# ZikangYuan/sr_livo

Hardware: AMD Instinct MI355X
Metric: sweeps/s (full ESIKF solve of a 64k-pt Livox sweep vs 1M-pt voxel map) (higher is better)
Workload: dtype f64; 1 GPU; HEADLINE: stream of 4 distinct 65536-keypoint livox sweeps (own poses and priors), 978481-pt voxel map (1000000 target), max_num_residuals=2147483647, r=1, K=20; one full ESIKF solve per sweep, every sweep crosses PCIe once (uploaded on the copy stream during the solve before it: resident in HBM when its solve starts); sweeps drawn with seeds 20251309 + 100 j, keeping those that take sweep 0's 2 E; parallelism=single GPU

## Files before the change

### sr_livo_amd/csrc/srl_capi.cpp

```cpp
#include "../../include/srlivo_hip.h"
#include "../../include/srlivo_hip_debug.h"
#include "host/srl_la.h"
#include "srl_device.h"
#include "srl_hash.h"
#include "srl_heap.h"

#include <hip/hip_runtime.h>
#include <sched.h>

#include <algorithm>
#include <atomic>
#include <chrono>
#include <climits>
#include <cstdio>
#include <cstdlib>
#include <cstring>
#include <mutex>
#include <string>
#include <vector>

struct SrlMapState;
int srl_map_insert_device(struct srl_ctx *ctx, const double *world_xyz, int n, double voxel_size, int cap,
                          double min_distance_points, int min_num_points, int *num_added);

// ... 135 lines not shown
    ctx->counted = true;
    *out = ctx;
    return SRL_OK;
}

int srl_ctx_destroy(srl_ctx *ctx) {
    if (!ctx) return SRL_OK;
    hipSetDevice(ctx->device);
    if (ctx->counted && ctx->device < SRL_MAX_DEVICES) g_live_ctx[ctx->device].fetch_sub(1, std::memory_order_relaxed);
    if (ctx->armed.on) srl_ctx_disarm(ctx);
    if (ctx->stream) hipStreamSynchronize(ctx->stream);
    if (ctx->copy_stream) hipStreamSynchronize(ctx->copy_stream);
    if (ctx->color) srl_color_map_destroy(ctx);
    if (ctx->flow) srl_flow_destroy(ctx);
    if (ctx->prep) srl_image_prep_destroy(ctx);
    srl_consensus_release(ctx);
    if (ctx->pose_box_pinned) hipHostFree(ctx->pose_box_pinned);
    if (ctx->pose_box_dev) hipFree(ctx->pose_box_dev);
    if (ctx->d_pose_relay) hipFree(ctx->d_pose_relay);
    if (ctx->comm && srl_rccl()) srl_rccl()->CommDestroy(ctx->comm);
    if (ctx->parked_comm && srl_rccl()) srl_rccl()->CommDestroy(ctx->parked_comm);
    if (ctx->d_sub_kept) hipFree(ctx->d_sub_kept);
    if (ctx->d_sub_seen) hipFree(ctx->d_sub_seen);
    void *bufs[] = {ctx->d_corr_in, ctx->d_corr_rel, ctx->d_corr_imu, ctx->d_corr_raw, ctx->d_corr_seg, ctx->d_frame_raw, ctx->d_frame_world, ctx->d_table, ctx->d_slabs, ctx->cur.soa, ctx->d_rec, ctx->d_status, ctx->d_partials, ctx->d_binfo,
                    ctx->d_out, ctx->d_count, ctx->d_bound, ctx->d_granules, ctx->d_rec_granules, ctx->next.soa, ctx->next.stage, ctx->cur.stage, ctx->d_tap_ids, ctx->d_tap_ncand, ctx->d_tap_normal, ctx->d_tap_a2d,
                    ctx->d_tap_offset, ctx->d_gather, ctx->d_peer, ctx->d_mail};
    for (int r = 0; r < SRL_MAX_PEERS; r++) if (ctx->peer_mapped[r]) hipIpcCloseMemHandle(ctx->peer_mapped[r]);
    if (ctx->d_inbox) hipFree(ctx->d_inbox);
    for (void *b : bufs) if (b) hipFree(b);
    if (ctx->h_out) hipHostFree(ctx->h_out);
    if (ctx->h_count) hipHostFree(ctx->h_count);
    if (ctx->h_mail) hipHostFree(ctx->h_mail);
    if (ctx->h_arm_stamps) hipHostFree(ctx->h_arm_stamps);
    if (ctx->h_scratch) hipHostFree(ctx->h_scratch);
    if (ctx->h_frame_x) hipHostFree(ctx->h_frame_x);
    for (SrlEpochTable *t : {&ctx->sel_table, &ctx->ins_table}) { if (t->keyw) hipFree(t->keyw); if (t->minw) hipFree(t->minw); }
    if (ctx->d_frame_sync) hipFree(ctx->d_frame_sync);
    if (ctx->d_tr1_sched) hipFree(ctx->d_tr1_sched);
    if (ctx->h_insert_cnt) hipHostFree(ctx->h_insert_cnt);
    if (ctx->ev_insert) hipEventDestroy(ctx->ev_insert);
    if (ctx->ev_world) hipEventDestroy(ctx->ev_world);
    if (ctx->ev_frame_read) hipEventDestroy(ctx->ev_frame_read);
    if (ctx->h_chunks) { hipHostFree(ctx->h_chunks); for (int i = 0; i < srl_ctx::CHUNK_SLOTS; i++) if (ctx->chunk_ev[i]) hipEventDestroy(ctx->chunk_ev[i]); }
    for (auto &b : ctx->pool_free) hipFree(b.p);
    ctx->pool_free.clear();
    for (int i = 0; i < 4; i++) if (ctx->ev[i]) hipEventDestroy(ctx->ev[i]);
    for (SrlProfRing::Entry &e : ctx->prof.e) for (int k = 0; k < 2; k++) if (e.ev[k]) hipEventDestroy(e.ev[k]);
    for (int sl = 0; sl < 2; sl++) for (int k = 0; k < 2; k++) if (ctx->up_ev[sl][k]) hipEventDestroy(ctx->up_ev[sl][k]);
    if (ctx->upload_ev) hipEventDestroy(ctx->upload_ev);
    if (ctx->copy_stream) { hipStreamSynchronize(ctx->copy_stream); hipStreamDestroy(ctx->copy_stream); }
    if (ctx->prefix_stream) { hipStreamSynchronize(ctx->prefix_stream); hipStreamDestroy(ctx->prefix_stream); }
    if (ctx->stream) hipStreamDestroy(ctx->stream);
    delete ctx;
    return SRL_OK;
}

const char *srl_last_error(const srl_ctx *ctx) { return ctx ? ctx->err.c_str() : "null context"; }

int srl_map_upload(srl_ctx *ctx, const int16_t *keys_xyz, const int32_t *counts, const float *xyz, int V, int cap) {
    if (!ctx || V < 0 || (V > 0 && (!keys_xyz || !counts || !xyz))) return SRL_ERR_BAD_ARG;
    SRL_DISARM(ctx);
    if (cap != SRL_VOXEL_CAP) { ctx->err = "max_num_points_in_voxel must be 20"; return SRL_ERR_UNSUPPORTED; }
    HIPCHK(ctx, hipSetDevice(ctx->device));
    { const int rcs = srl_map_settle(ctx); if (rcs) return rcs; }
    ctx->bound_n = 0;
    const unsigned slab_cap = std::max<unsigned>(1024u, (unsigned)V + (unsigned)V / 2u + 4096u);
    if (slab_cap > SRL_MAX_SLABS) { ctx->err = "map too large: slab byte offsets are 32-bit (16.7 M voxels)"; return SRL_ERR_UNSUPPORTED; }
    const unsigned table_cap = next_pow2(std::max<unsigned>(2048u, SRL_TABLE_FACTOR * slab_cap));
    std::vector<SrlSlab> slabs((size_t)V);
    std::vector<SrlMapSlot> table((size_t)table_cap);
    for (auto &s : table) { s.key = SRL_EMPTY_KEY; s.slab = 0; s.count = 0; }
    long long npts = 0;
    const unsigned mask = table_cap - 1;
    for (int v = 0; v < V; v++) {
        SrlSlab &s = slabs[v];
        std::memset(&s, 0, sizeof s);
        const int c = counts[v];
        if (c < 0 || c > cap) { ctx->err = "voxel count out of range"; return SRL_ERR_BAD_ARG; }
        for (int i = 0; i < c; i++)
            for (int d = 0; d < 3; d++) s.xyz[i][d] = xyz[((size_t)v * cap + i) * 3 + d];
        s.count = (unsigned)c;
        s.key = srl_pack_key(keys_xyz[3 * v], keys_xyz[3 * v + 1], keys_xyz[3 * v + 2]);
        npts += c;
        unsigned h = srl_hash_key(s.key) & mask;
        while (table[h].key != SRL_EMPTY_KEY) {
            if (table[h].key == s.key) { ctx->err = "duplicate voxel key in upload"; return SRL_ERR_BAD_ARG; }
            h = (h + 1) & mask;
        }
        table[h].key = s.key;
        table[h].slab = (unsigned)v;
        table[h].count = (unsigned)c;
    }
    if (ctx->d_slabs) { HIPCHK(ctx, hipFree(ctx->d_slabs)); ctx->d_slabs = nullptr; }
    if (ctx->d_table) { HIPCHK(ctx, hipFree(ctx->d_table)); ctx->d_table = nullptr; }
    HIPCHK(ctx, hipMalloc((void **)&ctx->d_slabs, ((size_t)slab_cap + 1) * SRL_SLAB_BYTES));
    HIPCHK(ctx, hipMemsetD32Async((hipDeviceptr_t)(ctx->d_slabs + (size_t)slab_cap * SRL_SLAB_BYTES), 0x7f800000, SRL_SLAB_BYTES / 4, ctx->stream));
    HIPCHK(ctx, hipMalloc((void **)&ctx->d_table, (size_t)table_cap * sizeof(SrlMapSlot)));
    HIPCHK(ctx, hipMemsetAsync(ctx->d_slabs, 0, (size_t)slab_cap * SRL_SLAB_BYTES, ctx->stream));
    if (V > 0) HIPCHK(ctx, hipMemcpyAsync(ctx->d_slabs, slabs.data(), (size_t)V * SRL_SLAB_BYTES, hipMemcpyHostToDevice, ctx->stream));
    HIPCHK(ctx, hipMemcpyAsync(ctx->d_table, table.data(), (size_t)table_cap * sizeof(SrlMapSlot), hipMemcpyHostToDevice, ctx->stream));
    HIPCHK(ctx, hipStreamSynchronize(ctx->stream));
    ctx->slab_cap = slab_cap;
    ctx->table_cap = table_cap;
    ctx->num_voxels = V;
    ctx->num_points = npts;
    return SRL_OK;
}

int srl_map_size(srl_ctx *ctx, int64_t *num_points, int32_t *num_voxels) {
    if (!ctx) return SRL_ERR_BAD_ARG;
    { const int rcs = srl_map_settle(ctx); if (rcs) return rcs; }
    if (num_points) *num_points = ctx->num_points;
    if (num_voxels) *num_voxels = ctx->num_voxels;
    return SRL_OK;
}

int srl_map_download(srl_ctx *ctx, int16_t *keys_xyz, int32_t *counts, float *xyz, int max_voxels) {
    if (!ctx) return SRL_ERR_BAD_ARG;
    SRL_DISARM(ctx);
    if (!ctx->d_slabs) return SRL_ERR_NO_MAP;
    { const int rcs = srl_map_settle(ctx); if (rcs) return rcs; }
    const int V = ctx->num_voxels;
    if (max_voxels < V) return SRL_ERR_BAD_ARG;
    HIPCHK(ctx, hipSetDevice(ctx->device));
    std::vector<SrlSlab> slabs((size_t)V);
    if (V > 0) HIPCHK(ctx, hipMemcpyAsync(slabs.data(), ctx->d_slabs, (size_t)V * SRL_SLAB_BYTES, hipMemcpyDeviceToHost, ctx->stream));
    HIPCHK(ctx, hipStreamSynchronize(ctx->stream));
    for (int v = 0; v < V; v++) {
        short x, y, z;
        srl_unpack_key(slabs[v].key, &x, &y, &z);
        if (keys_xyz) { keys_xyz[3 * v] = x; keys_xyz[3 * v + 1] = y; keys_xyz[3 * v + 2] = z; }
        if (counts) counts[v] = (int32_t)slabs[v].count;
        if (xyz)
            for (int i = 0; i < SRL_CAP; i++)
                for (int d = 0; d < 3; d++)
                    xyz[((size_t)v * SRL_CAP + i) * 3 + d] = (i < (int)slabs[v].count) ? slabs[v].xyz[i][d] : 0.0f;
    }
    return SRL_OK;
}

int srl_map_insert(srl_ctx *ctx, const double *world_xyz, int n, double voxel_size, int cap,
                   double min_distance_points, int min_num_points, int *num_added) {
    if (!ctx || n < 0 || (n > 0 && !world_xyz)) return SRL_ERR_BAD_ARG;
    SRL_DISARM(ctx);
    if (cap != SRL_VOXEL_CAP) { ctx->err = "max_num_points_in_voxel must be 20"; return SRL_ERR_UNSUPPORTED; }
    return srl_map_insert_device(ctx, world_xyz, n, voxel_size, cap, min_distance_points, min_num_points, num_added);
}

int srl_map_insert_report(srl_ctx *ctx, const double *world_xyz, int n, double voxel_size, int cap, double min_distance_points, int min_num_points,
                          double ref_z, uint8_t *outcome, srl_cloud_point *cloud, int *num_cloud, int *num_added) {
    if (num_cloud) *num_cloud = 0;
    if (num_added) *num_added = 0;
    if (!ctx || n < 0 || (n > 0 && !world_xyz)) return SRL_ERR_BAD_ARG;
    SRL_DISARM(ctx);
    if (cap != SRL_VOXEL_CAP) { ctx->err = "max_num_points_in_voxel must be 20"; return SRL_ERR_UNSUPPORTED; }
    return srl_map_insert_report_device(ctx, world_xyz, n, voxel_size, cap, min_distance_points, min_num_points, ref_z, outcome, cloud, num_cloud, num_added);
}

namespace {
int upload_aos(srl_ctx *ctx, const char *src, size_t bytes, double *d_stage, hipStream_t st, bool last = true, int pinned = -1) {
    if (pinned < 0 ? srl_is_pinned(src) : pinned != 0) {
        HIPCHK(ctx, hipMemcpyAsync(d_stage, src, bytes, hipMemcpyHostToDevice, st));
        if (last) {
            if (!ctx->upload_ev) HIPCHK(ctx, hipEventCreateWithFlags(&ctx->upload_ev, hipEventDisableTiming));
            HIPCHK(ctx, hipEventRecord(ctx->upload_ev, st));
            ctx->upload_pending = true;
        }
        return SRL_OK;
    }
    int rc2 = upload_chunks_init(ctx);
    if (rc2) return rc2;
// ... 1547 lines not shown
```

### sr_livo_amd/csrc/srl_hash.h

```cpp
#pragma once
#include <stdint.h>
#ifdef __HIPCC__
#define SRL_HD __host__ __device__
#else
#define SRL_HD
#endif

SRL_HD inline unsigned long long srl_pack_key(short x, short y, short z) {
    return (unsigned long long)(unsigned short)x | ((unsigned long long)(unsigned short)y << 16) |
           ((unsigned long long)(unsigned short)z << 32);
}
SRL_HD inline void srl_unpack_key(unsigned long long k, short *x, short *y, short *z) {
    *x = (short)(unsigned short)(k & 0xFFFFu);
    *y = (short)(unsigned short)((k >> 16) & 0xFFFFu);
    *z = (short)(unsigned short)((k >> 32) & 0xFFFFu);
}
SRL_HD inline unsigned srl_hash_key(unsigned long long k) {
    const unsigned x = (unsigned)(k & 0xFFFFu), y = (unsigned)((k >> 16) & 0xFFFFu), z = (unsigned)((k >> 32) & 0xFFFFu);
#ifdef __HIP_DEVICE_COMPILE__
    unsigned h = __umul24(x, 0x9E3779u) ^ __umul24(y, 0x85EBCBu) ^ __umul24(z, 0xC2B2AFu);
#else
    unsigned h = (x * 0x9E3779u) ^ (y * 0x85EBCBu) ^ (z * 0xC2B2AFu);
#endif
    h ^= h >> 15;
    h *= 0x2C1B3C6Du;
    h ^= h >> 12;
    return h;
}
```

### sr_livo_amd/csrc/srl_kernels.hip

```cpp
#include "srl_device.h"
#include "srl_hash.h"
#include "srl_heap.h"

#include <math.h>
#include <type_traits>

namespace {

struct alignas(8) VoxEnt { unsigned slab; unsigned count; };
struct Surv { double d2; float x, y, z; unsigned id; };
static_assert(sizeof(Surv) == 24, "survivor record is 24 bytes");
static_assert(SRL_SURV_CAP * 24 + (SRL_MAXK + 1) * 8 <= SRL_WAVE_SCRATCH, "general-path scratch (survivors + sorted d2) must fit");
static_assert(64 * 8 + SRL_MAXK * 16 + SRL_MAXK * 4 <= SRL_WAVE_SCRATCH, "heap replay scratch must fit");

__device__ __forceinline__ int lane_id() {
    return __builtin_amdgcn_mbcnt_hi(~0u, __builtin_amdgcn_mbcnt_lo(~0u, 0));
}
__device__ __forceinline__ int lanes_below(unsigned long long m) {
    return __builtin_amdgcn_mbcnt_hi((unsigned)(m >> 32), __builtin_amdgcn_mbcnt_lo((unsigned)m, 0));
}

struct Cand { bool valid; double d2; float x, y, z; unsigned id; };

__device__ __forceinline__ Cand eval_cand(int e, int nv, const VoxEnt *vox, const unsigned char *slabs,
                                          double qx, double qy, double qz) {
    Cand c;
    c.valid = false;
    c.d2 = __builtin_huge_val();
    c.x = c.y = c.z = 0.0f;
    c.id = 0;
    const unsigned cv = (unsigned)e / SRL_CAP;
    const unsigned slot = (unsigned)e - cv * SRL_CAP;
    if ((int)cv < nv) {
        const VoxEnt ve = vox[cv];
        if (slot < ve.count) {
            const float *p = reinterpret_cast<const float *>(slabs + (size_t)ve.slab * SRL_SLAB_BYTES + slot * 12u);
            c.x = p[0]; c.y = p[1]; c.z = p[2];
            const double dx = (double)c.x - qx;
            const double dy = (double)c.y - qy;
            const double dz = (double)c.z - qz;
            c.d2 = (dx * dx + dy * dy) + dz * dz;
            c.valid = true;
            c.id = ve.slab * SRL_CAP + slot;
        }
    }
    return c;
}

template <int NB>
__device__ __forceinline__ int probe_voxels(double qx, double qy, double qz, double size_voxel, int thr_cap,
                                            const SrlMapSlot *table, unsigned mask, VoxEnt *vox, int lane, const float *qf_cull = nullptr,
                                            int *total_all = nullptr) {
    constexpr int SIDE = 2 * NB + 1;
    constexpr int NV = SIDE * SIDE * SIDE;
    asm volatile("" : "+v"(lane));
    const short kx = (short)(int)(qx / size_voxel);
    const short ky = (short)(int)(qy / size_voxel);
    const short kz = (short)(int)(qz / size_voxel);
    int nv = 0, tot = 0;
#pragma unroll
    for (int base = 0; base < NV; base += 64) {
        const int i = base + lane;
        bool found = false;
        unsigned slab = 0, cnt = 0;
        float bd2 = 0.0f;
        if (i < NV) {
            const int ix = i / (SIDE * SIDE);
            const int iy = (i / SIDE) % SIDE;
            const int iz = i % SIDE;
            const short vx = (short)(kx + (ix - NB));
            const short vy = (short)(ky + (iy - NB));
            const short vz = (short)(kz + (iz - NB));
            const unsigned long long key = srl_pack_key(vx, vy, vz);
            unsigned h = srl_hash_key(key) & mask;
            for (unsigned probe = 0; probe <= mask; ++probe) {
                const SrlMapSlot s = table[h];
                if (s.key == key) {
                    found = (int)s.count >= thr_cap && s.count > 0;
                    slab = s.slab;
                    cnt = s.count;
                    break;
                }
                if (s.key == SRL_EMPTY_KEY) break;
                h = (h + 1) & mask;
            }
            if (qf_cull) {
                const int vv[3] = {(int)vx, (int)vy, (int)vz};
                const float sz = (float)size_voxel;
#pragma unroll
                for (int ax = 0; ax < 3; ++ax) {
                    const int v = vv[ax];
                    const float lo = (float)(v > 0 ? v : v - 1) * sz, hi = (float)(v < 0 ? v : v + 1) * sz;
                    const float d = fmaxf(fmaxf(lo - qf_cull[ax], qf_cull[ax] - hi), 0.0f);
                    bd2 += d * d;
                }
            }
        }
        tot += found ? (int)cnt : 0;
        if (qf_cull) found = found && bd2 <= qf_cull[5];
        const unsigned long long m = __ballot(found);
        if (found) {
            VoxEnt ve; ve.slab = slab; ve.count = cnt;
            vox[nv + lanes_below(m)] = ve;
        }
        nv += __popcll(m);
    }
    if (total_all) {
        for (int d = 32; d >= 1; d >>= 1) tot += __shfl_xor(tot, d);
        *total_all = tot;
    }
    __builtin_amdgcn_wave_barrier();
    return nv;
}

enum { SEL_OVERFLOW = 0, SEL_DONE = 1, SEL_TIE = 2 };
#define SRL_NEAR_TIE 0x1.0000000000004p+0

template <class Sink>
__device__ __forceinline__ void select_topk_replay(double qx, double qy, double qz, int nv, const VoxEnt *vox,
                                                const unsigned char *slabs, int K, void *scratch, int lane, Sink &sink,
                                                int &total_out) {
    double *stage = reinterpret_cast<double *>(scratch);
    double *hd = stage + 64;
    int *he = reinterpret_cast<int *>(hd + SRL_MAXK);
    int *out = he + SRL_MAXK;
    const int rounds = (nv * SRL_CAP + 63) >> 6;
    int size = 0, total = 0;
    __builtin_amdgcn_wave_barrier();
    for (int j = 0; j < rounds; ++j) {
        const Cand c = eval_cand(lane + 64 * j, nv, vox, slabs, qx, qy, qz);
        stage[lane] = c.valid ? sqrt(c.d2) : -1.0;
        total += __popcll(__ballot(c.valid));
        __builtin_amdgcn_wave_barrier();
        if (lane == 0) {
            for (int i = 0; i < 64; ++i) {
                const double d = stage[i];
                if (d >= 0.0) size = srl_heap_offer(hd, he, size, K, d, 64 * j + i);
            }
        }
        __builtin_amdgcn_wave_barrier();
    }
    if (lane == 0) srl_heap_drain(hd, he, size, out);
    __builtin_amdgcn_wave_barrier();
    size = __shfl(size, 0);
    if (lane < size) {
        const Cand c = eval_cand(out[lane], nv, vox, slabs, qx, qy, qz);
        sink.put(lane, c.x, c.y, c.z, c.id);
    }
    total_out = total;
    __builtin_amdgcn_wave_barrier();
}

template <class Sink>
__device__ __forceinline__ void select_topk(double qx, double qy, double qz, int nv, const VoxEnt *vox,
                                            const unsigned char *slabs, int K, int select_mode, Surv *surv,
                                            int lane, Sink &sink, int &total_out, int &fallback_out) {
    const int rounds = (nv * SRL_CAP + 63) >> 6;
    const float kInfF = __builtin_huge_valf();
    asm volatile("" : "+v"(lane));
    if (select_mode == 5) {
        select_topk_replay(qx, qy, qz, nv, vox, slabs, K, surv, lane, sink, total_out);
        fallback_out = 1;
        return;
    }

    float lmin = kInfF;
    int total = 0;
// ... 44 lines not shown

    if (!use_fallback) {
        const int i = lane;
        const bool act = i < c_surv;
        Surv me;
        if (act) me = surv[i];
        else { me.d2 = __builtin_huge_val(); me.x = me.y = me.z = 0.0f; me.id = 0; }
        int rank = 0;
        for (int j = 0; j < c_surv; ++j) {
            const double dj = surv[j].d2;
            rank += ((dj < me.d2) || (dj == me.d2 && j < i)) ? 1 : 0;
        }
        if (act && rank <= K) sorted[rank] = me.d2;
        __builtin_amdgcn_wave_barrier();
        bool bad = false;
        if (act && rank < K && rank + 1 < c_surv) bad = !(sorted[rank + 1] > me.d2 * SRL_NEAR_TIE);
        tie = __ballot(bad) != 0ull;
        if (!tie && act && rank < K) sink.put(rank, me.x, me.y, me.z, me.id);
        fallback_out = 0;
    } else {
        double last_d2 = -1.0;
        int last_e = -1;
        const int next = total < K + 1 ? total : K + 1;
        for (int r = 0; r < next; ++r) {
            double bd2 = __builtin_huge_val();
            int be = 0x7fffffff;
            for (int j = 0; j < rounds; ++j) {
                const int e = lane + 64 * j;
                const Cand c = eval_cand(e, nv, vox, slabs, qx, qy, qz);
                const bool gt = c.valid && (c.d2 > last_d2 || (c.d2 == last_d2 && e > last_e));
                if (gt && (c.d2 < bd2 || (c.d2 == bd2 && e < be))) { bd2 = c.d2; be = e; }
            }
#pragma unroll
            for (int off = 32; off >= 1; off >>= 1) {
                const double od = __shfl_xor(bd2, off);
                const int oe = __shfl_xor(be, off);
                if (od < bd2 || (od == bd2 && oe < be)) { bd2 = od; be = oe; }
            }
            if (r > 0 && !(bd2 > last_d2 * SRL_NEAR_TIE)) { tie = true; break; }
            if (r < nsel && (be & 63) == lane) {
                const Cand c = eval_cand(be, nv, vox, slabs, qx, qy, qz);
                sink.put(r, c.x, c.y, c.z, c.id);
            }
            last_d2 = bd2;
            last_e = be;
        }
        fallback_out = 1;
    }
    __builtin_amdgcn_wave_barrier();
    if (tie) {
        select_topk_replay(qx, qy, qz, nv, vox, slabs, K, surv, lane, sink, total_out);
        fallback_out = 1;
    }
}

struct LaneRole {
    int pdx, pdy, pdz;
    int c0, slot;
};
__device__ __forceinline__ LaneRole lane_role(int lane) {
    LaneRole r;
    const int pl = lane & 31;
    const int ix = pl / 9, iy = (pl / 3) % 3, iz = pl % 3;
    r.pdx = ix - 1; r.pdy = iy - 1; r.pdz = iz - 1;
    r.c0 = lane / SRL_CAP;
    r.slot = lane - r.c0 * SRL_CAP;
    return r;
}

struct ProbeReq {
    unsigned long long key;
    unsigned h;
    SrlMapSlot s0, s1;
};
__device__ __forceinline__ ProbeReq probe_issue(const int *kv, int kl, const LaneRole &role, const SrlMapSlot *table,
                                                unsigned mask, int lane) {
    ProbeReq r;
    r.key = SRL_EMPTY_KEY; r.h = 0;
    r.s0.key = SRL_EMPTY_KEY; r.s0.slab = 0; r.s0.count = 0;
    r.s1 = r.s0;
    if ((lane & 31) < 27) {
        const int *k = kv + (kl + (lane >> 5)) * 4;
        r.key = srl_pack_key((short)(k[0] + role.pdx), (short)(k[1] + role.pdy), (short)(k[2] + role.pdz));
        r.h = srl_hash_key(r.key) & mask;
        r.s0 = table[r.h];
        r.s1 = table[(r.h + 1) & mask];
    }
    return r;
}
__device__ __forceinline__ int probe_finish(const ProbeReq &r, int thr_cap, const SrlMapSlot *table, unsigned mask,
                                            VoxEnt *vox, int lane, int *ncand_pair, bool cull = false, const float *qf_pair = nullptr,
                                            const int *kv_pair = nullptr, const LaneRole *role = nullptr, float size_voxel = 1.0f) {
    const bool prober = (lane & 31) < 27;
    const bool m0 = prober && r.s0.key == r.key;
    const bool m1 = prober && !m0 && r.s0.key != SRL_EMPTY_KEY && r.s1.key == r.key;
    bool found = m0 || m1;
    unsigned slab = m0 ? r.s0.slab : r.s1.slab, cnt = m0 ? r.s0.count : r.s1.count;
    const bool more = prober && !found && r.s0.key != SRL_EMPTY_KEY && r.s1.key != SRL_EMPTY_KEY;
    if (__ballot(more) != 0ull) {
        if (more) {
            unsigned h = (r.h + 2) & mask;
            for (unsigned probe = 2; probe <= mask; ++probe) {
                const SrlMapSlot sl = table[h];
                if (sl.key == r.key) { slab = sl.slab; cnt = sl.count; found = true; break; }
                if (sl.key == SRL_EMPTY_KEY) break;
                h = (h + 1) & mask;
            }
        }
    }
    found = found && (int)cnt >= thr_cap && cnt > 0;
    {
#if defined(__HIP_DEVICE_COMPILE__)
        int v = found ? (int)cnt : 0;
        v += __builtin_amdgcn_update_dpp(0, v, 0x111, 0xF, 0xF, false);
        v += __builtin_amdgcn_update_dpp(0, v, 0x112, 0xF, 0xF, false);
        v += __builtin_amdgcn_update_dpp(0, v, 0x114, 0xF, 0xF, false);
        v += __builtin_amdgcn_update_dpp(0, v, 0x118, 0xF, 0xF, false);
        v += __builtin_amdgcn_update_dpp(0, v, 0x142, 0xA, 0xF, false);
        if ((lane & 31) == 31) ncand_pair[lane >> 5] = v;
#endif
    }
    if (cull) {
        const int hh = lane >> 5;
        const float *qf = qf_pair + 8 * hh;
        const int *kv = kv_pair + 4 * hh;
        const float r2 = qf[5];
        float bd2 = 0.0f;
        const int pd[3] = {role->pdx, role->pdy, role->pdz};
#pragma unroll
        for (int ax = 0; ax < 3; ++ax) {
            const int v = kv[ax] + pd[ax];
            const float lo = (float)(v > 0 ? v : v - 1) * size_voxel, hi = (float)(v < 0 ? v : v + 1) * size_voxel;
            const float d = fmaxf(fmaxf(lo - qf[ax], qf[ax] - hi), 0.0f);
            bd2 += d * d;
        }
        found = found && bd2 <= r2;
    }
    const unsigned long long m = __ballot(found);
    const unsigned m_lo = (unsigned)m, m_hi = (unsigned)(m >> 32);
    const int nv_a = __popc(m_lo), nv_b = __popc(m_hi);
    if (prober) {
        const bool upper = lane >= 32;
        const unsigned f_lo = found ? m_lo : (~m_lo & 0x7FFFFFFu), f_hi = found ? m_hi : (~m_hi & 0x7FFFFFFu);
        const int below = upper ? (int)__builtin_amdgcn_mbcnt_hi(f_hi, 0u) : (int)__builtin_amdgcn_mbcnt_lo(f_lo, 0u);
        const int nv_own = upper ? nv_b : nv_a;
        VoxEnt ve; ve.slab = found ? slab : 0u; ve.count = found ? cnt : 0u;
        vox[(upper ? 32 : 0) + (found ? below : nv_own + below)] = ve;
    }
    __builtin_amdgcn_wave_barrier();
    return nv_a | (nv_b << 8);
}

struct LdsSink {
    float *col;
    int row;
    int plane;
    int *tap_ids;
    __device__ __forceinline__ void put(int rank, float x, float y, float z, unsigned id) {
        float *p = col + rank * row;
        p[0] = x;
        p[plane] = y;
        p[2 * plane] = z;
        if (tap_ids) tap_ids[rank] = (int)id;
    }
};

struct alignas(16) SurvRec { float x, y, z; int code; };
#define SRL_PAIR_MAX_ROUNDS 4

__device__ __forceinline__ float d2_f32(float px, float py, float pz, float qx, float qy, float qz) {
#pragma clang fp contract(fast)
    const float dx = px - qx, dy = py - qy, dz = pz - qz;
    return dx * dx + dy * dy + dz * dz;
}

template <class Sink>
__device__ __forceinline__ int finish_survivors(double qx, double qy, double qz, int c, const VoxEnt *vox, int K, void *scratch,
                                                int lane, Sink &sink, double *tau_out = nullptr) {
    SurvRec *recs = reinterpret_cast<SurvRec *>(__builtin_assume_aligned(scratch, 16));
    double *keys = reinterpret_cast<double *>(reinterpret_cast<unsigned char *>(scratch) + 1024);
    double *sorted = keys + 66;
    __builtin_amdgcn_wave_barrier();
    const bool act = lane < c;
    SurvRec me;
    me.x = me.y = me.z = 0.0f; me.code = 0;
    double my = __builtin_huge_val();
    if (act) {
        me = recs[lane];
        const double dx = (double)me.x - qx;
// ... 1990 lines not shown
```

### sr_livo_amd/csrc/srl_map_kernels.hip

```cpp
#include "srl_ctx.h"
#include "srl_frame_scratch.h"
#include "srl_hash.h"


#include <cstring>
#include <vector>

namespace {


template <bool XF>
__global__ void k_point_slots(const double *xyz, int n, double voxel_size, unsigned long long *keyw, unsigned mask, unsigned epoch16, unsigned *slot_out,
                              unsigned *idx, int *new_flag, const SrlFrameTransform T) {
    const int i = blockIdx.x * blockDim.x + threadIdx.x;
    if (i >= n) return;
    double wx, wy, wz;
    if (XF) {
        srl_transform_point(T.X, T.raw[(size_t)i * 3], T.raw[(size_t)i * 3 + 1], T.raw[(size_t)i * 3 + 2], wx, wy, wz);
        T.world[(size_t)i * 3] = wx; T.world[(size_t)i * 3 + 1] = wy; T.world[(size_t)i * 3 + 2] = wz;
    } else {
        wx = xyz[(size_t)i * 3]; wy = xyz[(size_t)i * 3 + 1]; wz = xyz[(size_t)i * 3 + 2];
    }
    const float fx = (float)wx, fy = (float)wy, fz = (float)wz;
    const short kx = (short)(int)((double)fx / voxel_size);
    const short ky = (short)(int)((double)fy / voxel_size);
    const short kz = (short)(int)((double)fz / voxel_size);
    const unsigned long long key = srl_pack_key(kx, ky, kz);
    slot_out[i] = srl_epoch_claim(keyw, mask, epoch16, key, srl_hash_key(key));
    if (idx) idx[i] = (unsigned)i;
    new_flag[i] = 0;
}
struct HeadFlag32 {
    const unsigned *slots;
    __host__ __device__ int operator()(int i) const { return (i == 0 || slots[i] != slots[i - 1]) ? 1 : 0; }
};
struct SegmentSink {
    const unsigned *slots_sorted;
    const unsigned *idx_sorted;
    const unsigned long long *keyw;
    int *seg_start;
    unsigned long long *keys_sorted;
    const SrlMapSlot *table;
    unsigned mask;
    int *seg_slot;
    unsigned char *is_new;
    int *new_flag;
    int *seg_of_first;
    int *counters;
    int n;
    __device__ void operator()(int i, int head, int excl) const {
        if (head) {
            const unsigned long long key = keyw[slots_sorted[i]] & SRL_KEY48_MASK;
            keys_sorted[i] = key;
            seg_start[excl] = i;
            unsigned h = srl_hash_key(key) & mask;
            int slot = -1;
            for (unsigned probe = 0; probe <= mask; ++probe) {
                const unsigned long long k = table[h].key;
                if (k == key) { slot = (int)h; break; }
                if (k == SRL_EMPTY_KEY) break;
                h = (h + 1) & mask;
            }
            seg_slot[excl] = slot;
            is_new[excl] = slot < 0 ? 1 : 0;
            if (slot < 0 && new_flag) {
                const unsigned first = idx_sorted[i];
                new_flag[first] = 1;
                seg_of_first[first] = excl;
            }
        }
        if (i == n - 1) { counters[0] = excl + head; counters[1] = 0; counters[2] = 0; }
    }
};
struct CreateSink {
    const int *seg_of_first;
    const int *seg_start;
    const unsigned long long *keys_sorted;
    int V;
    SrlMapSlot *table;
    unsigned mask;
    unsigned char *slabs;
    int *seg_slot;
    int *counters;
    int n;
    __device__ void operator()(int i, int is_first_of_new, int rank) const {
        if (is_first_of_new) {
            const int s = seg_of_first[i];
            const unsigned long long key = keys_sorted[seg_start[s]];
            const unsigned slab = (unsigned)(V + rank);
            SrlSlab *sl = reinterpret_cast<SrlSlab *>(slabs + (size_t)slab * SRL_SLAB_BYTES);
            sl->count = 0;
            sl->pad = 0;
            sl->key = key;
            unsigned h = srl_hash_key(key) & mask;
            for (unsigned probe = 0; probe <= mask; ++probe) {
                const unsigned long long prev = atomicCAS(&table[h].key, SRL_EMPTY_KEY, key);
                if (prev == SRL_EMPTY_KEY) {
                    table[h].slab = slab;
                    table[h].count = 0;
                    seg_slot[s] = (int)h;
                    break;
                }
                h = (h + 1) & mask;
            }
        }
        if (i == n - 1) counters[1] = rank + is_first_of_new;
    }
};


__global__ void k_relookup(const int *seg_start, const unsigned long long *keys_sorted, const int *counters, const SrlMapSlot *table, unsigned mask,
                           int *seg_slot) {
    const int s = blockIdx.x * blockDim.x + threadIdx.x;
    if (s >= counters[0] || seg_slot[s] < 0) return;
    const unsigned long long key = keys_sorted[seg_start[s]];
    unsigned h = srl_hash_key(key) & mask;
    int slot = -1;
    for (unsigned probe = 0; probe <= mask; ++probe) {
        const unsigned long long k = table[h].key;
        if (k == key) { slot = (int)h; break; }
        if (k == SRL_EMPTY_KEY) break;
        h = (h + 1) & mask;
    }
    seg_slot[s] = slot;
}

struct SegmentSinkReport {
    SegmentSink base;
    unsigned char *outcome;
    __device__ void operator()(int i, int head, int excl) const {
        outcome[i] = 0;
        base(i, head, excl);
    }
};
struct OutcomeAppended {
    const unsigned char *outcome;
    __device__ int operator()(int i) const { return outcome[i] == 1 ? 1 : 0; }
};
struct CloudSink {
    const double *xyz;
    double ref_z;
    float4 *cloud;
    int *num_cloud;
    int n;
    __device__ void operator()(int i, int appended, int excl) const {
        if (appended) {
            const float fx = (float)xyz[(size_t)i * 3], fy = (float)xyz[(size_t)i * 3 + 1], fz = (float)xyz[(size_t)i * 3 + 2];
            cloud[excl] = make_float4(fx, fy, fz, (float)(50.0 * ((double)fz - ref_z)));
        }
        if (i == n - 1) *num_cloud = excl + appended;
    }
};


#define SRL_REPLAY_BATCH 8
template <bool REPORT>
__global__ void __launch_bounds__(128) k_replay(const int *seg_start, const unsigned *sorted_idx, const int *counters, int n, const double *xyz,
                         const int *seg_slot, const unsigned char *is_new, SrlMapSlot *table, unsigned char *slabs,
                         double voxel_size, double min_distance_points, int min_num_points, int *added_total, unsigned char *outcome) {
    const int s = blockIdx.x * blockDim.x + threadIdx.x;
    const int S = counters[0];
    if (s >= S) return;
    const int slot = seg_slot[s];
    if (slot < 0) return;
    const unsigned slab = table[slot].slab;
    SrlSlab *sl = reinterpret_cast<SrlSlab *>(slabs + (size_t)slab * SRL_SLAB_BYTES);
    int count = (int)sl->count;
    const bool fresh = is_new[s] != 0;
    const int j0 = seg_start[s], j1 = s + 1 < S ? seg_start[s + 1] : n;
    int added = 0;
    const double min_d2 = min_distance_points * min_distance_points;
    float sx[SRL_CAP], sy[SRL_CAP], sz[SRL_CAP];
#pragma unroll
    for (int k = 0; k < SRL_CAP; ++k) {
        const bool h = k < count;
        sx[k] = h ? sl->xyz[k][0] : 0.0f; sy[k] = h ? sl->xyz[k][1] : 0.0f; sz[k] = h ? sl->xyz[k][2] : 0.0f;
    }
    for (int jb = j0; jb < j1 && count < SRL_CAP; jb += SRL_REPLAY_BATCH) {
        unsigned idx[SRL_REPLAY_BATCH];
        float px[SRL_REPLAY_BATCH], py[SRL_REPLAY_BATCH], pz[SRL_REPLAY_BATCH];
#pragma unroll
        for (int b = 0; b < SRL_REPLAY_BATCH; ++b) idx[b] = sorted_idx[jb + b < j1 ? jb + b : j1 - 1];
#pragma unroll
        for (int b = 0; b < SRL_REPLAY_BATCH; ++b) {
            px[b] = (float)xyz[(size_t)idx[b] * 3]; py[b] = (float)xyz[(size_t)idx[b] * 3 + 1]; pz[b] = (float)xyz[(size_t)idx[b] * 3 + 2];
        }
#pragma unroll
        for (int b = 0; b < SRL_REPLAY_BATCH; ++b) {
            if (jb + b >= j1 || count == SRL_CAP) break;
            const float fx = px[b], fy = py[b], fz = pz[b];
            bool add;
            if (fresh && count == 0) {
                add = true;
            } else {
                double sq_dist_min = 10 * voxel_size * voxel_size;
#pragma unroll
                for (int k = 0; k < SRL_CAP; ++k) {
                    if (k < count) {
                        const double dx = (double)sx[k] - (double)fx;
                        const double dy = (double)sy[k] - (double)fy;
                        const double dz = (double)sz[k] - (double)fz;
                        const double sq = (dx * dx + dy * dy) + dz * dz;
                        if (sq < sq_dist_min) sq_dist_min = sq;
                    }
                }
                add = (sq_dist_min > min_d2) && (min_num_points <= 0 || count >= min_num_points);
            }
            if (REPORT) outcome[idx[b]] = add ? (fresh && count == 0 ? 2 : 1) : 0;
            if (add) {
                sl->xyz[count][0] = fx; sl->xyz[count][1] = fy; sl->xyz[count][2] = fz;
#pragma unroll
                for (int k = 0; k < SRL_CAP; ++k) if (k == count) { sx[k] = fx; sy[k] = fy; sz[k] = fz; }
                ++count;
                ++added;
            }
        }
    }
    sl->count = (unsigned)count;
    table[slot].count = (unsigned)count;
    if (added) atomicAdd(added_total, added);
}

__global__ void k_probe_checksum(const double *xyz, int n, int stride, double voxel_size, const SrlMapSlot *table, unsigned mask, const unsigned char *slabs,
                                 unsigned long long *sum) {
    const long long i = (long long)(blockIdx.x * blockDim.x + threadIdx.x) * stride;
    unsigned long long mine = 0ull;
    if (i < n) {
        const float fx = (float)xyz[(size_t)i * 3], fy = (float)xyz[(size_t)i * 3 + 1], fz = (float)xyz[(size_t)i * 3 + 2];
        const short kx = (short)(int)((double)fx / voxel_size), ky = (short)(int)((double)fy / voxel_size), kz = (short)(int)((double)fz / voxel_size);
        const unsigned long long key = srl_pack_key(kx, ky, kz);
        unsigned h = srl_hash_key(key) & mask;
        for (unsigned probe = 0; probe <= mask; ++probe) {
            const SrlMapSlot sl = table[h];
            if (sl.key == key) {
                const SrlSlab *sb = reinterpret_cast<const SrlSlab *>(slabs + (size_t)sl.slab * SRL_SLAB_BYTES);
                const int c = (int)sb->count;
                if (c > 0) mine = srl_probe_mix(kx, ky, kz, c, sb->xyz[c - 1][0], sb->xyz[c - 1][1], sb->xyz[c - 1][2]);
                break;
            }
            if (sl.key == SRL_EMPTY_KEY) break;
            h = (h + 1) & mask;
        }
    }
#pragma unroll
    for (int off = 32; off >= 1; off >>= 1) mine += __shfl_xor(mine, off);
    if ((threadIdx.x & 63) == 0 && mine != 0ull) atomicAdd(sum, mine);
}

__global__ void k_rebuild_table(const unsigned char *slabs, int V, SrlMapSlot *table, unsigned mask) {
    const int v = blockIdx.x * blockDim.x + threadIdx.x;
    if (v >= V) return;
    const SrlSlab *sl = reinterpret_cast<const SrlSlab *>(slabs + (size_t)v * SRL_SLAB_BYTES);
    const unsigned long long key = sl->key;
    unsigned h = srl_hash_key(key) & mask;
    for (unsigned probe = 0; probe <= mask; ++probe) {
        const unsigned long long prev = atomicCAS(&table[h].key, SRL_EMPTY_KEY, key);
        if (prev == SRL_EMPTY_KEY) { table[h].slab = (unsigned)v; table[h].count = sl->count; return; }
        h = (h + 1) & mask;
    }
}

__global__ void k_fill_empty(SrlMapSlot *table, unsigned cap) {
    const unsigned i = blockIdx.x * blockDim.x + threadIdx.x;
    if (i >= cap) return;
    SrlMapSlot s; s.key = SRL_EMPTY_KEY; s.slab = 0; s.count = 0;
    table[i] = s;
}

#define SRL_PRUNE_MARK_BLOCKS 1024
__global__ void __launch_bounds__(1024) k_prune_mark(const unsigned char *slabs, int V, double lx, double ly, double lz, double r2, int *keep,
                                                     unsigned long long *points_removed) {
    __shared__ unsigned long long wave_sum[16];
    unsigned long long mine = 0ull;
    for (int v = blockIdx.x * 1024 + threadIdx.x; v < V; v += gridDim.x * 1024) {
        const SrlSlab *sl = reinterpret_cast<const SrlSlab *>(slabs + (size_t)v * SRL_SLAB_BYTES);
        const double dx = (double)sl->xyz[0][0] - lx;
        const double dy = (double)sl->xyz[0][1] - ly;
        const double dz = (double)sl->xyz[0][2] - lz;
        const bool erase = (dx * dx + dy * dy) + dz * dz > r2;
        keep[v] = erase ? 0 : 1;
        if (erase) mine += sl->count;
    }
#pragma unroll
    for (int off = 32; off >= 1; off >>= 1) mine += __shfl_xor(mine, off);
    if ((threadIdx.x & 63) == 0) wave_sum[threadIdx.x >> 6] = mine;
    __syncthreads();
    if (threadIdx.x == 0) {
        unsigned long long s = 0ull;
        for (int w = 0; w < 16; ++w) s += wave_sum[w];
        if (s != 0ull) atomicAdd(points_removed, s);
    }
}
struct PruneRankSink {
    int *rank;
    int *survivors;
    int n;
    __device__ void operator()(int i, int keep, int excl) const {
        rank[i] = excl;
        if (i == n - 1) *survivors = excl + keep;
    }
};
__global__ void __launch_bounds__(256) k_prune_compact(const unsigned char *slabs, int V, const int *keep, const int *rank, unsigned char *dst) {
    const int v = blockIdx.x * 16 + (threadIdx.x >> 4);
    const int lane = threadIdx.x & 15;
    if (v >= V || !keep[v]) return;
    const uint4 *src = reinterpret_cast<const uint4 *>(slabs + (size_t)v * SRL_SLAB_BYTES);
    uint4 *out = reinterpret_cast<uint4 *>(dst + (size_t)rank[v] * SRL_SLAB_BYTES);
    out[lane] = src[lane];
}

unsigned next_pow2u(unsigned v) { unsigned p = 1; while (p < v) p <<= 1; return p; }

}

extern "C" int srl_map_remove_far(srl_ctx *ctx, const double location[3], double distance, int32_t *num_voxels_removed, int64_t *num_points_removed) {
    if (num_voxels_removed) *num_voxels_removed = 0;
    if (num_points_removed) *num_points_removed = 0;
    if (!ctx || !location) return SRL_ERR_BAD_ARG;
    SRL_DISARM(ctx);
    HIPCHK(ctx, hipSetDevice(ctx->device));
    { const int rcs = srl_map_settle(ctx); if (rcs) return rcs; }
    const int V = ctx->num_voxels;
    if (!ctx->d_table || V <= 0) return SRL_OK;
    hipStream_t st = ctx->stream;
    DevBuf b_keep, b_rank, b_cnt, b_sc;
    HIPCHK(ctx, b_keep.alloc(ctx, (size_t)V * 4));
    HIPCHK(ctx, b_rank.alloc(ctx, (size_t)V * 4));
    HIPCHK(ctx, b_cnt.alloc(ctx, 64));
    HIPCHK(ctx, b_sc.alloc(ctx, srl_scan_scratch_ints(V) * 4));
    unsigned long long *d_removed = b_cnt.as<unsigned long long>();
    int *d_surv = b_cnt.as<int>() + 2;
    HIPCHK(ctx, hipMemsetAsync(b_cnt.p, 0, 16, st));
    hipLaunchKernelGGL(k_prune_mark, dim3(std::min((V + 1023) / 1024, SRL_PRUNE_MARK_BLOCKS)), dim3(1024), 0, st, ctx->d_slabs, V, location[0], location[1],
                       location[2], distance * distance, b_keep.as<int>(), d_removed);
    HIPCHK(ctx, hipGetLastError());
    srl_scan(SrlIntArrayIn{b_keep.as<int>()}, PruneRankSink{b_rank.as<int>(), d_surv, V}, V, b_sc.as<int>(), st);
    HIPCHK(ctx, hipGetLastError());
    { const int rc = ensure_host_scratch(ctx, 64); if (rc) return rc; }
    HIPCHK(ctx, hipMemcpyAsync(ctx->h_scratch, b_cnt.p, 16, hipMemcpyDeviceToHost, st));
    HIPCHK(ctx, hipStreamSynchronize(st));
    long long pts_removed = 0;
// ... 279 lines not shown
```

Measured before the change: 11030 sweeps/s.

## Group 2x2x2 voxel neighborhoods into contiguous hash slots with strided probing

```diff
diff --git a/sr_livo_amd/csrc/srl_capi.cpp b/sr_livo_amd/csrc/srl_capi.cpp
--- a/sr_livo_amd/csrc/srl_capi.cpp
+++ b/sr_livo_amd/csrc/srl_capi.cpp
@@ -241,11 +241,10 @@
         s.count = (unsigned)c;
         s.key = srl_pack_key(keys_xyz[3 * v], keys_xyz[3 * v + 1], keys_xyz[3 * v + 2]);
         npts += c;
-        unsigned h = srl_hash_key(s.key) & mask;
-        while (table[h].key != SRL_EMPTY_KEY) {
+        const unsigned home = srl_table_home(s.key, mask);
+        unsigned h = home;
+        for (unsigned probe = 0; table[h].key != SRL_EMPTY_KEY; h = srl_table_slot(home, ++probe, mask))
             if (table[h].key == s.key) { ctx->err = "duplicate voxel key in upload"; return SRL_ERR_BAD_ARG; }
-            h = (h + 1) & mask;
-        }
         table[h].key = s.key;
         table[h].slab = (unsigned)v;
         table[h].count = (unsigned)c;
diff --git a/sr_livo_amd/csrc/srl_hash.h b/sr_livo_amd/csrc/srl_hash.h
--- a/sr_livo_amd/csrc/srl_hash.h
+++ b/sr_livo_amd/csrc/srl_hash.h
@@ -15,8 +15,7 @@
     *y = (short)(unsigned short)((k >> 16) & 0xFFFFu);
     *z = (short)(unsigned short)((k >> 32) & 0xFFFFu);
 }
-SRL_HD inline unsigned srl_hash_key(unsigned long long k) {
-    const unsigned x = (unsigned)(k & 0xFFFFu), y = (unsigned)((k >> 16) & 0xFFFFu), z = (unsigned)((k >> 32) & 0xFFFFu);
+SRL_HD inline unsigned srl_mix_xyz(unsigned x, unsigned y, unsigned z) {
 #ifdef __HIP_DEVICE_COMPILE__
     unsigned h = __umul24(x, 0x9E3779u) ^ __umul24(y, 0x85EBCBu) ^ __umul24(z, 0xC2B2AFu);
 #else
@@ -27,3 +26,23 @@
     h ^= h >> 12;
     return h;
 }
+SRL_HD inline unsigned srl_hash_key(unsigned long long k) {
+    return srl_mix_xyz((unsigned)(k & 0xFFFFu), (unsigned)((k >> 16) & 0xFFFFu), (unsigned)((k >> 32) & 0xFFFFu));
+}
+
+SRL_HD inline unsigned srl_table_home(unsigned long long k, unsigned mask) {
+    const unsigned x = (unsigned)(k & 0xFFFFu), y = (unsigned)((k >> 16) & 0xFFFFu), z = (unsigned)((k >> 32) & 0xFFFFu);
+    const unsigned sub = (x & 1u) | ((y & 1u) << 1) | ((z & 1u) << 2);
+    return ((srl_mix_xyz(x >> 1, y >> 1, z >> 1) << 3) | sub) & mask;
+}
+SRL_HD inline unsigned srl_table_log2(unsigned mask) {
+#ifdef __HIP_DEVICE_COMPILE__
+    return (unsigned)__popc(mask);
+#else
+    return (unsigned)__builtin_popcount(mask);
+#endif
+}
+SRL_HD inline unsigned srl_table_slot(unsigned home, unsigned i, unsigned mask) {
+    const unsigned s = i << 3;
+    return (home + s + (s >> srl_table_log2(mask))) & mask;
+}
diff --git a/sr_livo_amd/csrc/srl_kernels.hip b/sr_livo_amd/csrc/srl_kernels.hip
--- a/sr_livo_amd/csrc/srl_kernels.hip
+++ b/sr_livo_amd/csrc/srl_kernels.hip
@@ -72,9 +72,9 @@
             const short vy = (short)(ky + (iy - NB));
             const short vz = (short)(kz + (iz - NB));
             const unsigned long long key = srl_pack_key(vx, vy, vz);
-            unsigned h = srl_hash_key(key) & mask;
+            const unsigned home = srl_table_home(key, mask);
             for (unsigned probe = 0; probe <= mask; ++probe) {
-                const SrlMapSlot s = table[h];
+                const SrlMapSlot s = table[srl_table_slot(home, probe, mask)];
                 if (s.key == key) {
                     found = (int)s.count >= thr_cap && s.count > 0;
                     slab = s.slab;
@@ -82,7 +82,6 @@
                     break;
                 }
                 if (s.key == SRL_EMPTY_KEY) break;
-                h = (h + 1) & mask;
             }
             if (qf_cull) {
                 const int vv[3] = {(int)vx, (int)vy, (int)vz};
@@ -293,9 +292,9 @@
     if ((lane & 31) < 27) {
         const int *k = kv + (kl + (lane >> 5)) * 4;
         r.key = srl_pack_key((short)(k[0] + role.pdx), (short)(k[1] + role.pdy), (short)(k[2] + role.pdz));
-        r.h = srl_hash_key(r.key) & mask;
+        r.h = srl_table_home(r.key, mask);
         r.s0 = table[r.h];
-        r.s1 = table[(r.h + 1) & mask];
+        r.s1 = table[srl_table_slot(r.h, 1u, mask)];
     }
     return r;
 }
@@ -310,12 +309,10 @@
     const bool more = prober && !found && r.s0.key != SRL_EMPTY_KEY && r.s1.key != SRL_EMPTY_KEY;
     if (__ballot(more) != 0ull) {
         if (more) {
-            unsigned h = (r.h + 2) & mask;
             for (unsigned probe = 2; probe <= mask; ++probe) {
-                const SrlMapSlot sl = table[h];
+                const SrlMapSlot sl = table[srl_table_slot(r.h, probe, mask)];
                 if (sl.key == r.key) { slab = sl.slab; cnt = sl.count; found = true; break; }
                 if (sl.key == SRL_EMPTY_KEY) break;
-                h = (h + 1) & mask;
             }
         }
     }
diff --git a/sr_livo_amd/csrc/srl_map_kernels.hip b/sr_livo_amd/csrc/srl_map_kernels.hip
--- a/sr_livo_amd/csrc/srl_map_kernels.hip
+++ b/sr_livo_amd/csrc/srl_map_kernels.hip
@@ -53,13 +53,13 @@
             const unsigned long long key = keyw[slots_sorted[i]] & SRL_KEY48_MASK;
             keys_sorted[i] = key;
             seg_start[excl] = i;
-            unsigned h = srl_hash_key(key) & mask;
+            const unsigned home = srl_table_home(key, mask);
             int slot = -1;
             for (unsigned probe = 0; probe <= mask; ++probe) {
+                const unsigned h = srl_table_slot(home, probe, mask);
                 const unsigned long long k = table[h].key;
                 if (k == key) { slot = (int)h; break; }
                 if (k == SRL_EMPTY_KEY) break;
-                h = (h + 1) & mask;
             }
             seg_slot[excl] = slot;
             is_new[excl] = slot < 0 ? 1 : 0;
@@ -92,8 +92,9 @@
             sl->count = 0;
             sl->pad = 0;
             sl->key = key;
-            unsigned h = srl_hash_key(key) & mask;
+            const unsigned home = srl_table_home(key, mask);
             for (unsigned probe = 0; probe <= mask; ++probe) {
+                const unsigned h = srl_table_slot(home, probe, mask);
                 const unsigned long long prev = atomicCAS(&table[h].key, SRL_EMPTY_KEY, key);
                 if (prev == SRL_EMPTY_KEY) {
                     table[h].slab = slab;
@@ -101,7 +102,6 @@
                     seg_slot[s] = (int)h;
                     break;
                 }
-                h = (h + 1) & mask;
             }
         }
         if (i == n - 1) counters[1] = rank + is_first_of_new;
@@ -114,13 +114,13 @@
     const int s = blockIdx.x * blockDim.x + threadIdx.x;
     if (s >= counters[0] || seg_slot[s] < 0) return;
     const unsigned long long key = keys_sorted[seg_start[s]];
-    unsigned h = srl_hash_key(key) & mask;
+    const unsigned home = srl_table_home(key, mask);
     int slot = -1;
     for (unsigned probe = 0; probe <= mask; ++probe) {
+        const unsigned h = srl_table_slot(home, probe, mask);
         const unsigned long long k = table[h].key;
         if (k == key) { slot = (int)h; break; }
         if (k == SRL_EMPTY_KEY) break;
-        h = (h + 1) & mask;
     }
     seg_slot[s] = slot;
 }
@@ -229,9 +229,9 @@
         const float fx = (float)xyz[(size_t)i * 3], fy = (float)xyz[(size_t)i * 3 + 1], fz = (float)xyz[(size_t)i * 3 + 2];
         const short kx = (short)(int)((double)fx / voxel_size), ky = (short)(int)((double)fy / voxel_size), kz = (short)(int)((double)fz / voxel_size);
         const unsigned long long key = srl_pack_key(kx, ky, kz);
-        unsigned h = srl_hash_key(key) & mask;
+        const unsigned home = srl_table_home(key, mask);
         for (unsigned probe = 0; probe <= mask; ++probe) {
-            const SrlMapSlot sl = table[h];
+            const SrlMapSlot sl = table[srl_table_slot(home, probe, mask)];
             if (sl.key == key) {
                 const SrlSlab *sb = reinterpret_cast<const SrlSlab *>(slabs + (size_t)sl.slab * SRL_SLAB_BYTES);
                 const int c = (int)sb->count;
@@ -239,7 +239,6 @@
                 break;
             }
             if (sl.key == SRL_EMPTY_KEY) break;
-            h = (h + 1) & mask;
         }
     }
 #pragma unroll
@@ -252,11 +251,11 @@
     if (v >= V) return;
     const SrlSlab *sl = reinterpret_cast<const SrlSlab *>(slabs + (size_t)v * SRL_SLAB_BYTES);
     const unsigned long long key = sl->key;
-    unsigned h = srl_hash_key(key) & mask;
+    const unsigned home = srl_table_home(key, mask);
     for (unsigned probe = 0; probe <= mask; ++probe) {
+        const unsigned h = srl_table_slot(home, probe, mask);
         const unsigned long long prev = atomicCAS(&table[h].key, SRL_EMPTY_KEY, key);
         if (prev == SRL_EMPTY_KEY) { table[h].slab = (unsigned)v; table[h].count = sl->count; return; }
-        h = (h + 1) & mask;
     }
 }
 
```

New measurement: 10790 sweeps/s. 0.978x the previous value.
